# ekinakyurek/Long-Term-Recurrent-Convolutional-NN

Hardware: AMD Instinct MI355X
Metric: training images/sec (VGG16+LSTM, COCO, batch 256) at 1/2/4/8 MI355X (higher is better)
Workload: dtype bf16

## Files before the change

long-term-recurrent-convolutional-nn_amd/_lib.py:

```python
import ctypes as C
import os
import subprocess

HERE = os.path.dirname(os.path.abspath(__file__))
CSRC = os.path.join(HERE, "csrc")
LIB_PATH = os.environ.get("LRCN_HIP_LIB") or os.path.join(CSRC, "liblrcn_hip.so")
HEADER = os.path.normpath(os.path.join(HERE, "..", "include", "lrcn.h"))
SAMPLE_HEADER = os.path.normpath(os.path.join(HERE, "..", "include", "lrcn_sample.h"))
SCORE_HEADER = os.path.normpath(os.path.join(HERE, "..", "include", "lrcn_score.h"))
NUCLEUS_HEADER = os.path.normpath(os.path.join(HERE, "..", "include", "lrcn_nucleus.h"))
NBEST_HEADER = os.path.normpath(os.path.join(HERE, "..", "include", "lrcn_nbest.h"))
DIVERSE_HEADER = os.path.normpath(os.path.join(HERE, "..", "include", "lrcn_diverse.h"))
CONSTRAIN_HEADER = os.path.normpath(os.path.join(HERE, "..", "include", "lrcn_constrain.h"))
ACTIVITY_HEADER = os.path.normpath(os.path.join(HERE, "..", "include", "lrcn_activity.h"))
ACT_DROPOUT_HEADER = os.path.normpath(os.path.join(HERE, "..", "include", "lrcn_act_dropout.h"))
VARLEN_HEADER = os.path.normpath(os.path.join(HERE, "..", "include", "lrcn_varlen.h"))
CLIP_HEADER = os.path.normpath(os.path.join(HERE, "..", "include", "lrcn_clip.h"))
WEIGHTED_HEADER = os.path.normpath(os.path.join(HERE, "..", "include", "lrcn_weighted.h"))
SCHED_HEADER = os.path.normpath(os.path.join(HERE, "..", "include", "lrcn_sched.h"))
SMOOTH_HEADER = os.path.normpath(os.path.join(HERE, "..", "include", "lrcn_smooth.h"))
GEMM_DEBUG_HEADER = os.path.normpath(os.path.join(HERE, "..", "include", "lrcn_gemm_debug.h"))
CONV_DEBUG_HEADER = os.path.normpath(os.path.join(HERE, "..", "include", "lrcn_conv_debug.h"))
DECODE_DEBUG_HEADER = os.path.normpath(os.path.join(HERE, "..", "include", "lrcn_decode_debug.h"))

LRCN_F32, LRCN_BF16, LRCN_FP8 = 0, 1, 2
LRCN_ABI_VERSION = 5
LRCN_OPT_FUSED_UPDATE, LRCN_OPT_DETERMINISTIC, LRCN_OPT_CONV_CHUNK_BYTES = 1, 2, 3
SEGMENTS = ("update", "rec_fwd", "rec_bwd", "embed_gather", "embed_grad", "preprocess", "upload")
EOS, BOS, UNK = 0, 1, 2
CNNOUT = 4096
MAX_T = 28


class LrcnError(RuntimeError):
    pass


class Config(C.Structure):
# ... 256 lines not shown
    "lrcn_debug_conv_gemm": (C.c_int, [C.c_void_p, C.POINTER(ConvGemmDebug)]),
}

CONV_DEBUG_SIGNATURES = {
    "lrcn_debug_conv11": (C.c_int, [C.c_void_p, C.c_void_p, C.c_int, C.c_int, C.c_int, C.POINTER(C.c_float), C.c_void_p, C.c_void_p, C.c_void_p]),
    "lrcn_debug_fp8_cast": (C.c_int, [C.c_void_p, C.c_int, C.c_void_p, C.c_int64, C.c_float, C.c_void_p]),
    "lrcn_debug_amax": (C.c_int, [C.c_void_p, C.c_void_p, C.c_int64, C.c_void_p]),
    "lrcn_debug_conv64_f8": (C.c_int, [C.c_void_p, C.c_void_p, C.c_int, C.c_int, C.c_int, C.c_void_p, C.c_void_p, C.c_int, C.c_float, C.c_void_p]),
    "lrcn_debug_fp8_scales": (C.c_int, [C.c_void_p, C.POINTER(C.c_float)]),
}

DECODE_DEBUG_SIGNATURES = {
    "lrcn_debug_decode_steps": (C.c_int, [C.c_void_p, C.POINTER(DecodeDebug)]),
}


def build(force=False):
    srcs = [os.path.join(CSRC, f) for f in os.listdir(CSRC) if f.endswith((".hip", ".h"))] + [HEADER, SAMPLE_HEADER, NUCLEUS_HEADER, SCORE_HEADER, NBEST_HEADER, DIVERSE_HEADER, CONSTRAIN_HEADER,
                                                                                                   ACTIVITY_HEADER, ACT_DROPOUT_HEADER, VARLEN_HEADER, CLIP_HEADER, WEIGHTED_HEADER, SCHED_HEADER, SMOOTH_HEADER, GEMM_DEBUG_HEADER, CONV_DEBUG_HEADER, DECODE_DEBUG_HEADER]
    stale = force or not os.path.exists(LIB_PATH) or os.path.getmtime(LIB_PATH) < max(os.path.getmtime(s) for s in srcs)
    if stale:
        subprocess.check_call(["make", "-s", "-j4", "-C", CSRC, "-f", os.path.join(CSRC, "Makefile")])
    return LIB_PATH


_LIB = None


def lib():
    global _LIB
    if _LIB is None:
        if not os.path.exists(LIB_PATH):
            raise LrcnError("%s is missing: run `python -c 'import __graft_entry__ as g; g.build()'` "
                            "(there is no CPU fallback)" % LIB_PATH)
        import torch
        L = C.CDLL(LIB_PATH)
        for name, (res, args) in list(SIGNATURES.items()) + list(SAMPLE_SIGNATURES.items()) + list(NUCLEUS_SIGNATURES.items()) + list(SCORE_SIGNATURES.items()) + list(NBEST_SIGNATURES.items()) + list(DIVERSE_SIGNATURES.items()) + list(CONSTRAIN_SIGNATURES.items()) + \
                list(ACTIVITY_SIGNATURES.items()) + list(ACT_DROPOUT_SIGNATURES.items()) + list(VARLEN_SIGNATURES.items()) + list(CLIP_SIGNATURES.items()) + list(WEIGHTED_SIGNATURES.items()) + list(SCHED_SIGNATURES.items()) + list(SMOOTH_SIGNATURES.items()) + \
                list(GEMM_DEBUG_SIGNATURES.items()) + list(CONV_DEBUG_SIGNATURES.items()) + list(DECODE_DEBUG_SIGNATURES.items()):
            fn = getattr(L, name)
            fn.restype = res
            fn.argtypes = args
        if L.lrcn_abi_version() != LRCN_ABI_VERSION:
            raise LrcnError("%s implements ABI revision %d, this binding was written against %d (lrcn_config's layout differs)"
                            % (LIB_PATH, L.lrcn_abi_version(), LRCN_ABI_VERSION))
        _LIB = L
    return _LIB


def check(ctx_handle, rc):
    if rc != 0:
        msg = lib().lrcn_last_error(ctx_handle)
        raise LrcnError("liblrcn_hip error %d: %s" % (rc, msg.decode() if msg else "?"))
```

long-term-recurrent-convolutional-nn_amd/csrc/ctx.h:

```cpp
#pragma once
#include <utility>

#include "comm.h"
#include "host.h"
#include "../../include/lrcn_smooth.h"

namespace lrcn_impl {

struct VggLayer {
    void *w = nullptr;
    void *w_fused = nullptr;
    float *b = nullptr;
    int Cin = 0, Cout = 0, S = 0, pool = 0;
    void *w8 = nullptr;
    float *sw = nullptr, *escale = nullptr, *ebias = nullptr;
};
constexpr int kFp8First = 3;

}

struct lrcn_ctx {
    lrcn_config cfg{};
    hipStream_t stream = nullptr;
    std::string err;
// ... 81 lines not shown
    void *cn_arena = nullptr;
    size_t cn_bytes = 0;
    void *sc_arena = nullptr;
    size_t sc_bytes = 0;
    int ncu = 0;
    int vgg_wg_cap = 0;
    bool vgg_loaded = false;
    bool vgg_fp8 = false, fp8_ready = false;
    float *amax_dev = nullptr;
    float act_scale[13] = {};
    lrcn_impl::VggLayer conv[13];
    void *fc6w = nullptr, *fc7w = nullptr;
    float *fc6b = nullptr, *fc7b = nullptr;
    void *actA = nullptr, *actB = nullptr, *im2col = nullptr, *f6 = nullptr, *img16 = nullptr;
    float *featsRM = nullptr;
    bool prof = false;
    std::vector<std::pair<hipEvent_t, hipEvent_t>> prof_ev;
    size_t prof_used = 0;
    double prof_ms = 0.0;
    int64_t prof_launches = 0;
    int prof_level = 0;
    struct SegProf {
        std::vector<std::pair<hipEvent_t, hipEvent_t>> ev;
        size_t used = 0;
        double ms = 0.0, bytes = 0.0;
        int64_t n = 0;
    } seg[LRCN_SEG_COUNT];
    std::string vgg_routes;
    float *avg_img = nullptr;
    bool avg_on = false;
// ... 106 lines not shown
```

long-term-recurrent-convolutional-nn_amd/csrc/lrcn_api.hip:

```cpp
#include <algorithm>
#include <cmath>

#include "ctx.h"

static thread_local std::string g_create_err;
using namespace lrcn_impl;

constexpr int kBgWgsPerFreeCu = 4;

int lrcn_impl::gemm(lrcn_ctx *c, int dtype, const void *A, int64_t lda, const void *B, int64_t ldb, void *C, int64_t ldc, int M, int N,
         int K, const float *bias, bool c_f32, bool beta, bool relu, bool c_is_zero, bool on_wg_stream) {
    GemmArgs g{};
    g.dtype = dtype;
    g.A = A;
    g.lda = lda;
    g.B = B;
    g.ldb = ldb;
    g.C = C;
    g.ldc = ldc;
    g.M = M;
    g.N = N;
    g.K = gemm_k(dtype, lda, ldb, K);
    g.bias = bias;
    g.c_f32 = c_f32;
// ... 134 lines not shown
    if (c->wg_done) (void)hipEventDestroy(c->wg_done);
    if (c->xc_fork) (void)hipEventDestroy(c->xc_fork);
    if (c->xc_done) (void)hipEventDestroy(c->xc_done);
    if (c->pin) (void)hipHostFree(c->pin);
    if (c->lens_pin) (void)hipHostFree(c->lens_pin);
    for (auto &e : c->lens_up)
        if (e) (void)hipEventDestroy(e);
    if (c->roww_pin) (void)hipHostFree(c->roww_pin);
    for (auto &e : c->roww_up)
        if (e) (void)hipEventDestroy(e);
    if (c->wg_stream && c->wg_stream_owned) (void)hipStreamDestroy(c->wg_stream);
    if (c->copy_stream) (void)hipStreamDestroy(c->copy_stream);
    for (int j = 0; j < lrcn_ctx::kStage; ++j) {
        if (c->up_done[j]) (void)hipEventDestroy(c->up_done[j]);
        if (c->rd_done[j]) (void)hipEventDestroy(c->rd_done[j]);
    }
    comm_destroy(c->comm);
    for (auto &e : c->bucket_done)
        if (e) (void)hipEventDestroy(e);
    for (auto &e : c->ar_done)
        if (e) (void)hipEventDestroy(e);
    if (c->comm_stream && c->comm_stream_owned) (void)hipStreamDestroy(c->comm_stream);
    for (auto &sp : c->seg)
        for (auto &e : sp.ev) {
            (void)hipEventDestroy(e.first);
            (void)hipEventDestroy(e.second);
        }
    for (auto &e : c->prof_ev) {
        (void)hipEventDestroy(e.first);
        (void)hipEventDestroy(e.second);
// ... 324 lines not shown
```

long-term-recurrent-convolutional-nn_amd/csrc/train.hip:

```cpp
#include <cmath>
#include <cstring>

#include "ctx.h"
#include "../../include/lrcn_varlen.h"
#include "../../include/lrcn_clip.h"
#include "../../include/lrcn_weighted.h"
#include "../../include/lrcn_sched.h"
#include "../../include/lrcn_smooth.h"

using namespace lrcn_impl;

namespace {

DropSpec make_drop(const lrcn_dropout *d, int which) {
    DropSpec s{};
    s.which = which;
    if (d) {
        s.p = d->pdrop;
        s.seed = d->seed;
        s.mask = which == 1 ? d->mask1 : d->mask2;
        if (s.mask) s.p = 0.0f;
    }
    return s;
}
// ... 63 lines not shown
            g.out_mode = GEMM_OUT_LSTM_BWD;
            g.lstm.H = H; g.lstm.ld_a = ld4H;
            g.lstm.acts = const_cast<char *>(boff(acts, (int64_t)(s - 1) * B * ld4H, c->esz));
            g.lstm.c_prev = s > 1 ? Call + (int64_t)(s - 2) * B * H : nullptr;
            g.lstm.c_new = Call + (int64_t)(s - 1) * B * H;
            g.lstm.dh_ext = dHall + (int64_t)(s - 1) * B * H;
            g.lstm.dc = c->dc;
            g.lstm.dz_out = boff(dZ, (int64_t)(s - 1) * B * ld4H, c->esz);
            hipError_t e = launch_gemm_8p(c->stream, g);
            if (e != hipSuccess) FAIL(c, LRCN_EHIP, "lstm bwd step (GEMM + cell epilogue): %s", hipGetErrorString(e));
        }
        KCHK(c, "lstm_layer_bwd (epilogue)");
        return LRCN_OK;
    }
    {
        const int nsl = knob_int("LRCN_BWD_SLABS", 0);
        const int Kp = (int)round_up64(4 * H, 64);
        if (!fused && nsl >= 2 && nsl <= 8 && dt == GEMM_T_BF16 && !lstm_alone(c) && bg_row_window(B) && !(H & 3) && H >= 128 &&
            Kp / 64 >= 8 * nsl && Kp <= ld4H && (size_t)nsl * B * H * sizeof(float) <= c->gemm_ws_bytes && c->gemm_ws) {
            float *slabs = reinterpret_cast<float *>(c->gemm_ws);
            for (int s = S - 1; s >= 0; --s) {
                k_lstm_bwd(c->stream, dt, boff(acts, (int64_t)s * B * ld4H, c->esz), ld4H, s ? Call + (int64_t)(s - 1) * B * H : nullptr,
                           Call + (int64_t)s * B * H, dHall + (int64_t)s * B * H, H, slabs, s < S - 1, c->dc, s == S - 1, B, H,
                           boff(dZ, (int64_t)s * B * ld4H, c->esz), ld4H, nsl);
                if (s > 0) {
                    GemmArgs g = rec_step_args(c, dZ, ld4H, s, B, WhT, H, Kp);
                    g.C = slabs; g.ldc = H; g.c_f32 = 1;
                    g.out_mode = GEMM_OUT_PLAIN;
                    g.ws = c->gemm_ws; g.ws_bytes = c->gemm_ws_bytes;
                    g.cfg_pref = 2;
                    g.splitk_forced = 1; g.splitk_no_reduce = 1;
// ... 600 lines not shown
```

long-term-recurrent-convolutional-nn_amd/csrc/vgg.hip:

```cpp
#include <algorithm>
#include <cstring>

#include "ctx.h"
#include "../../include/lrcn_conv_debug.h"
#include "../../include/lrcn_gemm_debug.h"

using namespace lrcn_impl;

static const int kVggCout[13] = {64, 64, 128, 128, 256, 256, 256, 512, 512, 512, 512, 512, 512};
static const int kVggPool[13] = {0, 1, 0, 1, 0, 0, 1, 0, 0, 1, 0, 0, 1};

namespace {
int stamps_reserve(lrcn_ctx *c, int64_t need) {
    if (need > c->stamps_n) {
        c->stamps = nullptr;
        DALLOC(c, c->stamps, sizeof(unsigned long long) * (size_t)need);
        c->stamps_n = need;
    }
    return LRCN_OK;
}
bool conv64_enabled() { return !knob_off("LRCN_CONV64"); }
constexpr int kTileCtrStride = 8 + 2 * 512;
hipError_t launch_conv_chunked(hipStream_t st, const GemmArgs &g0, int N, int es, int64_t limit_bytes = 0) {
    const int64_t per_img = (int64_t)g0.H * g0.W * g0.Cin * es;
// ... 66 lines not shown

int conv_layer_fp8(lrcn_ctx *c, const void *in, const VggLayer &L, int N, void *out, int *tile_ctr = nullptr) {
    GemmArgs g = conv_args(c, GEMM_T_F8, in, L, N, out, tile_ctr);
    g.B = L.w8;
    g.bias = L.ebias;
    g.scale = L.escale;
    hipError_t e = launch_conv_chunked(c->stream, g, N, 1, c->conv_chunk_bytes > 0 ? c->conv_chunk_bytes : 0x7F000000ll);
    if (e != hipSuccess) FAIL(c, LRCN_EHIP, "fp8 conv layer S=%d Cin=%d Cout=%d: %s", L.S, L.Cin, L.Cout, hipGetErrorString(e));
    return LRCN_OK;
}

}

namespace lrcn_impl {

int vgg_body(lrcn_ctx *c, int N, const void *src, bool src_u8, const float *mean, bool calibrate) {
    const bool fp8 = c->vgg_fp8 && !calibrate;
    if (fp8 && !c->fp8_ready) FAIL(c, LRCN_ESTATE, "vgg_dtype = LRCN_FP8: call lrcn_vgg_calibrate before the first forward");
    const int vdt = c->vdt;
    const float m0 = mean ? mean[0] : 0.f, m1 = mean ? mean[1] : 0.f, m2 = mean ? mean[2] : 0.f;
    const bool fuse11 = vdt == GEMM_T_BF16 && src_u8 && c->conv[0].w_fused && conv64_enabled() && !knob_off("LRCN_FUSE11");
    const float *avg = (src_u8 && c->avg_on) ? c->avg_img : nullptr;
    int staged = -1;
    if (src_u8)
        for (int j = 0; j < lrcn_ctx::kStage; ++j)
            if (c->stage[j] && src == c->stage[j]) staged = j;
    if (staged >= 0) HIPCHK(c, hipStreamWaitEvent(c->stream, c->up_done[staged], 0));
    auto crops_consumed = [&]() -> int {
        if (staged < 0) return LRCN_OK;
        HIPCHK(c, hipEventRecord(c->rd_done[staged], c->stream));
        c->stage_read[staged] = true;
// ... 40 lines not shown
        g.out_mode = GEMM_OUT_CONV;
        g.H = g.W = 224;
        g.zero_page = c->zero_page;
        hipError_t e = launch_gemm(c->stream, g);
        if (e != hipSuccess) FAIL(c, LRCN_EHIP, "conv1_1: %s", hipGetErrorString(e));
    }
    if (int r = crops_consumed()) return r;
    if (!fuse11) note(vdt == GEMM_T_BF16 ? "conv11" : gemm_debug_last_route());
    void *cur = c->actA, *nxt = c->actB;
    int *ctr = nullptr;
    if (c->vgg_wg_cap >= 8 && knob_char("LRCN_DYN_TILES") == '1') {
        if (!c->tile_ctr) DALLOC(c, c->tile_ctr, sizeof(int) * 13 * kTileCtrStride);
        HIPCHK(c, hipMemsetAsync(c->tile_ctr, 0, sizeof(int) * 13 * kTileCtrStride, c->stream));
        ctr = c->tile_ctr;
    }
    std::pair<hipEvent_t, hipEvent_t> *ev = nullptr;
    if (c->prof) {
        if (c->prof_used == c->prof_ev.size()) {
            std::pair<hipEvent_t, hipEvent_t> e;
            HIPCHK(c, hipEventCreate(&e.first));
            HIPCHK(c, hipEventCreate(&e.second));
            c->prof_ev.push_back(e);
        }
        ev = &c->prof_ev[c->prof_used++];
        HIPCHK(c, hipEventRecord(ev->first, c->stream));
    }
    int l0 = 1;
    if (fuse11) {
        unsigned long long *stamps = nullptr;
        if (knob_char("LRCN_STAMPS") == 'f') {
            if (int r = stamps_reserve(c, (int64_t)N * 14 * 14 * 16)) return r;
            stamps = c->stamps;
        }
        hipError_t e = launch_conv64_fused11(c->stream, c->img16, c->conv[0].w_fused, c->conv[0].b, c->conv[1].w, c->conv[1].b, nxt, N, 224,
                                             c->zero_page, c->vgg_wg_cap, stamps);
        if (e != hipSuccess) FAIL(c, LRCN_EHIP, "fused conv1_1+conv1_2: %s", hipGetErrorString(e));
        note(gemm_debug_last_route());
        std::swap(cur, nxt);
        l0 = 2;
    }
    auto out_count = [&](int l) {
        const VggLayer &L = c->conv[l];
        const int64_t So = L.pool ? L.S / 2 : L.S;
        return (int64_t)N * So * So * L.Cout;
    };
    bool in_is_f8 = false;
    for (int l = l0; l < 13; ++l) {
        if (fp8 && l == kFp8First && !in_is_f8) {
            k_cast_bf16_fp8(c->stream, cur, out_count(l - 1), 1.0f / c->act_scale[l - 1], nxt);
            std::swap(cur, nxt);
        }
        int r;
        if (fp8 && l >= kFp8First)
            r = conv_layer_fp8(c, cur, c->conv[l], N, nxt, ctr ? ctr + l * kTileCtrStride : nullptr);
        else
            r = conv_layer(c, vdt, cur, c->conv[l], N, nxt, (fp8 && l == kFp8First - 1) ? 1.0f / c->act_scale[l] : 0.0f, &in_is_f8,
                           ctr ? ctr + l * kTileCtrStride : nullptr);
        if (r) return r;
        note(gemm_debug_last_route());
        std::swap(cur, nxt);
        if (calibrate && l >= kFp8First - 1) k_amax(c->stream, cur, out_count(l), c->amax_dev + l);
    }
    if (fp8) {
        k_cast_fp8_bf16(c->stream, cur, out_count(12), c->act_scale[12], nxt);
        std::swap(cur, nxt);
    }
    if (ev) HIPCHK(c, hipEventRecord(ev->second, c->stream));
    GemmArgs g{};
    g.dtype = vdt;
    g.A = cur;
    g.lda = 25088;
    g.B = c->fc6w;
    g.ldb = 25088;
    g.M = N;
    g.N = 4096;
    g.K = 25088;
    g.zero_page = c->zero_page;
    g.ws = c->vgg_ws;
    g.ws_bytes = c->gemm_ws_bytes;
    g.C = c->f6;
    g.ldc = 4096;
    g.bias = c->fc6b;
    g.relu = 1;
    hipError_t e = launch_gemm(c->stream, g);
    if (e != hipSuccess) FAIL(c, LRCN_EHIP, "fc6: %s", hipGetErrorString(e));
    note(gemm_debug_last_route());
    g.A = c->f6;
    g.lda = 4096;
    g.B = c->fc7w;
    g.ldb = 4096;
    g.C = c->featsRM;
    g.K = 4096;
    g.bias = c->fc7b;
    g.relu = 0;
    g.c_f32 = 1;
    e = launch_gemm(c->stream, g);
    if (e != hipSuccess) FAIL(c, LRCN_EHIP, "fc7: %s", hipGetErrorString(e));
    note(gemm_debug_last_route());
    return LRCN_OK;
}
int vgg_check(lrcn_ctx *c, int N) {
    if (!c->vgg_loaded) FAIL(c, LRCN_ESTATE, "lrcn_vgg_load has not been called");
    if (N < 1 || N > c->cfg.max_images) FAIL(c, LRCN_EINVAL, "N=%d outside [1,%d]", N, c->cfg.max_images);
    return LRCN_OK;
}
}

extern "C" {

int lrcn_vgg_load(lrcn_ctx *c, const float *const cw[13], const float *const cb[13], const float *fc6_w, const float *fc6_b,
                  const float *fc7_w, const float *fc7_b) {
    DeviceGuard dg(c);
    if (!c || !cw || !cb || !fc6_w || !fc6_b || !fc7_w || !fc7_b) return LRCN_EINVAL;
    if (c->cfg.max_images < 1) FAIL(c, LRCN_ESTATE, "context was created with max_images = 0");
// ... 269 lines not shown
    if (!c || !img || !feats || (!mean && !c->avg_on)) return LRCN_EINVAL;
    int r = vgg_check(c, N);
    if (r) return r;
    if (block_rows < 1 || N % block_rows) FAIL(c, LRCN_EINVAL, "block_rows=%d must divide N=%d", block_rows, N);
    r = vgg_body(c, N, img, true, mean);
    if (r) return r;
    for (int b = 0; b < N / block_rows; ++b) {
        float *dst = feats + (int64_t)b * block_rows * LRCN_CNNOUT;
        k_transpose_f32(c->stream, c->featsRM + (int64_t)b * block_rows * LRCN_CNNOUT, 4096, block_rows, 4096, dst, block_rows);
        if (normalize) k_normalize_rows(c->stream, dst, block_rows, LRCN_CNNOUT);
    }
    KCHK(c, "vgg_forward_u8_blocks");
    return LRCN_OK;
}

int lrcn_preprocess_u8(lrcn_ctx *c, const uint8_t *img, int N, const float mean[3], float *out) {
    DeviceGuard dg(c);
    if (!c || !img || !out || (!mean && !c->avg_on) || N < 1) return LRCN_EINVAL;
    k_preprocess_u8(c->stream, img, N, 224, mean ? mean[0] : 0.f, mean ? mean[1] : 0.f, mean ? mean[2] : 0.f, c->avg_on ? c->avg_img : nullptr, out);
    KCHK(c, "preprocess_u8");
    return LRCN_OK;
}

int lrcn_set_average_image(lrcn_ctx *c, const float *avg) {
    DeviceGuard dg(c);
    if (!c) return LRCN_EINVAL;
    if (!avg) {
        c->avg_on = false;
        return LRCN_OK;
    }
// ... 337 lines not shown
```

long-term-recurrent-convolutional-nn_amd/dp.py:

```python
import collections
import ctypes as C
import os

import numpy as np
import torch
import torch.distributed as dist

from . import lrcn as L


def shard_rows(B_global, world, rank):
    if B_global % world:
        raise L.LrcnError("global batch %d is not divisible by world size %d" % (B_global, world))
    b = B_global // world
    return slice(rank * b, (rank + 1) * b)


def vgg_wg_cap_for(device, rows=256, chunk=1):
    ncu = torch.cuda.get_device_properties(device).multi_processor_count
    if chunk > 1 and rows <= 32:
        return (ncu * 5 // 8) & ~7
    if chunk > 1 and rows <= 64:
        return (ncu * 11 // 16) & ~7
    return (ncu * 7 // 8) & ~7
# ... 53 lines not shown

class HipOps:

    def __init__(self, ctx, mean=L.VGG_MEAN):
        self.ctx = ctx
        self.mean = mean

    def vgg(self, img_u8, feats=None, normalize=False):
        return L.convnet_u8(self.ctx, img_u8, mean=self.mean, feats=feats, normalize=normalize)

    def loss(self, param, feats, tokens, lens=None):
        return L.avg_loss_batch(self.ctx, param, feats, tokens, lens=lens)

    def vgg_blocks(self, img_u8, rows, feats=None, normalize=False):
        return L.convnet_u8_blocks(self.ctx, img_u8, rows, mean=self.mean, feats=feats, normalize=normalize)

    def upload(self, host_u8):
        return L.upload_crops(self.ctx, host_u8)

    def params_touched(self):
        self.ctx.params_touched()

    def side_stream(self):
        if os.environ.get("LRCN_OVERLAP_VGG", "1")[:1] == "0":
            return None
        prio = int(os.environ.get("LRCN_VGG_STREAM_PRIO", "0"))
        return torch.cuda.Stream(device=self.ctx.device, priority=prio)

    def set_vgg_wg_cap(self, cap):
        self.ctx._call("lrcn_vgg_set_wg_cap", int(cap))
# ... 144 lines not shown
            self._v = [torch.zeros(n, device=dev, dtype=torch.float32) for n in n_of]
            self._gshard = [torch.zeros(n, device=dev, dtype=torch.float32) for n in n_of]
            self._scatter_optim_state()
        else:
            self.flat_grads, self.grads = flat_model_like(shapes, device=param[0].device)
        self.step_no = 0
        self._feat_q = collections.deque()
        self._chunk_no = 0
        self._side = self.ops.side_stream() if hasattr(self.ops, "side_stream") else None
        if self._side is not None and hasattr(self.ops, "set_vgg_wg_cap"):
            env = os.environ.get("LRCN_VGG_WG_CAP")
            cap = int(env) if env is not None else vgg_wg_cap_for(param[0].device, int(rows) if rows else B_global // max(world, 1), int(vgg_chunk))
            self.ops.set_vgg_wg_cap(cap)
            self.vgg_cap = cap
        self._feats_buf = [None, None]
        if (self._side is not None and isinstance(self._side, torch.cuda.Stream) and ctx is not None and hasattr(self.ops, "set_wg_stream")
                and os.environ.get("LRCN_DP_WG_STREAM_PROBE", "1")[:1] != "0"):
            self.ops.set_wg_stream(avoid=[self._side, torch.cuda.current_stream(ctx.device)])
        self._bucket_streams = None
        self._abi_stream_set = False
        env_sp = os.environ.get("LRCN_DP_SPARSE_EMBED")
        want = (env_sp[:1] != "0") if env_sp else world > 1
        self._sparse_embed = bool(want and self.backend == "torch" and not self.shard and not host_clip and self._multi_or_forced_sparse(env_sp)
                                  and hasattr(self.ops, "embed_grad_from_rows") and hasattr(self.ops, "update_group") and ctx is not None
                                  and self._group_pipeline())
        if self._sparse_embed:
            W = max(world, 1)
            cap = (ctx.max_T + 1) * min(ctx.max_B, int(rows) if rows else ctx.max_B)
            if W * cap > 8192:
                self._sparse_embed = False
# ... 203 lines not shown
        return self.ops.vgg(img_u8, normalize=True) if self.normalize_features else self.ops.vgg(img_u8)

    def _vgg_blocks(self, img_u8, rows, out=None):
        if img_u8.shape[0] == rows or not hasattr(self.ops, "vgg_blocks"):
            if img_u8.shape[0] != rows:
                raise L.LrcnError("crops for %d rows given, the step has %d (these ops cannot run several batches in one forward)" % (img_u8.shape[0], rows))
            return [self.ops.vgg(img_u8, feats=out, normalize=True) if self.normalize_features else self.ops.vgg(img_u8, feats=out)]
        if img_u8.shape[0] % rows:
            raise L.LrcnError("crops for %d rows are not a whole number of %d-row batches" % (img_u8.shape[0], rows))
        return self.ops.vgg_blocks(img_u8, rows, feats=out, normalize=self.normalize_features)

    def _vgg_on_side_stream(self, img_u8, rows):
        main = torch.cuda.current_stream(self.ctx.device)
        k = self._chunk_no & 1
        self._chunk_no += 1
        n = img_u8.shape[0] * L.CNNOUT
        if self._feats_buf[k] is None or self._feats_buf[k].numel() != n:
            self._feats_buf[k] = (torch.empty(n, device=self.param[0].device, dtype=torch.float32) if img_u8.shape[0] != rows
                                  else L.jl_empty(rows, L.CNNOUT))
        self._side.wait_stream(main)
        self.ctx.use_stream(self._side)
        try:
            blocks = self._vgg_blocks(img_u8, rows, out=self._feats_buf[k])
        finally:
            self.ctx.use_stream(main)
        if torch.is_tensor(img_u8) and img_u8.is_cuda:
            img_u8.record_stream(self._side)
        ev = torch.cuda.Event()
        ev.record(self._side)
        for b in blocks:
# ... 17 lines not shown
        if label_smoothing > 0:
            if self.backend == "abi" and self._multi:
                raise L.LrcnError("the \"abi\" data-parallel backend (lrcn_train_step_dp) has no label smoothing; use backend=\"torch\"")
            if lens is None:
                lens = np.full(rows, int(tokens.shape[0]), np.int32)
                norm_tokens = self.B_global * (int(tokens.shape[0]) + 1)
        if sched is not None:
            if self.backend == "abi" and self._multi:
                raise L.LrcnError("the \"abi\" data-parallel backend (lrcn_train_step_dp) has no scheduled sampling; use backend=\"torch\"")
            eps, temperature, sseed = tuple(sched)[:3]
            sched = (eps, temperature, sseed, shard_rows(self.B_global, self.world, self.rank).start)
            if lens is None:
                lens = np.full(rows, int(tokens.shape[0]), np.int32)
                norm_tokens = self.B_global * (int(tokens.shape[0]) + 1)
        self._cur_M = (int(tokens.shape[0]) + 1) * rows
        if feats is None:
            if self._feat_q:
                feats, ev = self._feat_q.popleft()
                if ev is not None:
                    torch.cuda.current_stream(self.ctx.device).wait_event(ev)
            else:
                blocks = self._vgg_blocks(self._device_crops(img_u8), rows)
                feats = blocks[0]
                self._feat_q.extend((b, None) for b in blocks[1:])
        self.step_no += 1
        consumed, deferred = False, None
        if next_img_u8 is not None and len(self._feat_q) < max(1, next_img_u8.shape[0] // rows):
            consumed = True
            nxt = self._device_crops(next_img_u8)
            if self._side is not None:
                self._vgg_on_side_stream(nxt, rows)
            else:
                deferred = nxt
            if prefetch_img_u8 is not None and hasattr(self.ops, "upload") and torch.is_tensor(prefetch_img_u8) and not prefetch_img_u8.is_cuda:
                self._prefetched = (prefetch_img_u8, self.ops.upload(prefetch_img_u8))

        def inorder_vgg():
            if deferred is not None:
                self._feat_q.extend((b, None) for b in self._vgg_blocks(deferred, rows))
# ... 158 lines not shown
            else:
                parts = [torch.empty_like(mine) for _ in range(self._W)]
                dist.all_gather(parts, mine.clone(), group=self.group)
                for i, t in enumerate(parts):
                    self.flat_param[a + i * n:a + (i + 1) * n].copy_(t)
        if self._shadow_groups:
            self.ops.refresh_shadows_group(self.param, k, s)

    def describe(self):
        buckets = os.environ.get("LRCN_DP_BUCKETS", "1")[:1] != "0"
        return {"backend": self.backend, "update": "sharded" if self.shard else "replicated", "fused_update": bool(self._fused),
                "shadows_by_group": bool(getattr(self, "_shadow_groups", False)),
                "per_group_pipeline": bool(self.shard or (self.backend == "abi" and self._multi) or self._group_pipeline()),
                "one_allreduce_of_the_flat_buffer": bool(self.world > 1 and not buckets and not self.shard),
                "sparse_embedding_exchange": bool(getattr(self, "_sparse_embed", False)), "vgg_side_stream": self._side is not None,
                "queue_probe": getattr(self, "queue_probe", None), "backend_note": self.backend_note or None,
                "update_stream_on_its_own_queue": getattr(self.ops, "update_stream_probed", None)}

    def _dist_on(self):
        return dist.is_available() and dist.is_initialized()

    def _gather_cat(self, t):
        if not self._dist_on():
            return t.clone()
        W = dist.get_world_size(self.group)
        if dist.get_backend(self.group) == "nccl":
            out = torch.empty((W,) + tuple(t.shape), device=t.device, dtype=t.dtype)
            dist.all_gather_into_tensor(out, t.contiguous(), group=self.group)
            return out.view((W * t.shape[0],) + tuple(t.shape[1:]))
        h = t.detach().cpu().contiguous()
# ... 84 lines not shown
```

long-term-recurrent-convolutional-nn_amd/launch.py:

```python
import json
import os
import signal
import socket
import subprocess
import sys
import tempfile
import time


def find_free_port():
    with socket.socket() as sk:
        sk.bind(("127.0.0.1", 0))
        return sk.getsockname()[1]


def run_ranks(script, argv, nranks, env_extra=None, watchdog_s=900.0, capture=True):
    env = dict(os.environ)
    env.setdefault("HSA_ENABLE_IPC_MODE_LEGACY", "0")
    env.update(env_extra or {})
    cmd = [sys.executable, "-m", "torch.distributed.run", "--nnodes=1", "--nproc-per-node", str(nranks), "--master-addr", "127.0.0.1",
           "--master-port", str(find_free_port()), os.path.abspath(script)] + list(argv)
    proc = subprocess.Popen(cmd, env=env, stdout=subprocess.PIPE if capture else None, stderr=None, text=True, start_new_session=True)

    def stop_job():
# ... 20 lines not shown
            rc = proc.returncode
        except subprocess.TimeoutExpired:
            stop_job()
            out, _ = proc.communicate()
            rc = 124
    finally:
        stop_job()
        for sg, h in old.items():
            signal.signal(sg, h)
    return rc, out


PLAIN_ENV = {
    "LRCN_DP_BACKEND": "torch", "LRCN_DP_SHARD_ADAM": "0", "LRCN_DP_SPARSE_EMBED": "0", "LRCN_DP_BUCKETS": "0", "LRCN_DP_GROUP_ADAM": "0",
    "LRCN_DP_QUEUE_PROBE": "0", "LRCN_DP_WG_STREAM_PROBE": "0", "LRCN_FUSED_UPDATE": "0", "LRCN_VGG_CHUNK_IMAGES": "0",
}


def default_rungs(dp_backend="torch"):
    rungs = []
    if dp_backend == "auto":
        rungs.append(("abi", {"LRCN_DP_BACKEND": "abi"}))
    rungs.append(("default", {"LRCN_DP_BACKEND": "abi" if dp_backend == "abi" else "torch"}))
    rungs.append(("plain", dict(PLAIN_ENV)))
    return rungs


def _set_pdeathsig():
    try:
        import ctypes
# ... 176 lines not shown
```

long-term-recurrent-convolutional-nn_amd/lrcn.py:

```python
import ctypes as C

import numpy as np
import torch

from . import _lib
from ._lib import BOS, CNNOUT, EOS, LRCN_BF16, LRCN_F32, LRCN_FP8, UNK, LrcnError

PARAM_NAMES = ("W1", "b1", "W2", "b2", "Wproj", "Wcnn", "Wembed", "Wout", "bout")
VGG_COUT = (64, 64, 128, 128, 256, 256, 256, 512, 512, 512, 512, 512, 512)
VGG_MEAN = (123.68, 116.779, 103.939)


def jl_empty(*dims, device="cuda", dtype=torch.float32):
    t = torch.empty(tuple(reversed(dims)), device=device, dtype=dtype)
    return t.permute(*reversed(range(len(dims))))


def jl_zeros(*dims, device="cuda", dtype=torch.float32):
    t = jl_empty(*dims, device=device, dtype=dtype)
    t.zero_()
    return t


def to_jl(a, device="cuda"):
# ... 739 lines not shown


def convnet_u8_blocks(ctx, img_u8, block_rows, mean=VGG_MEAN, feats=None, normalize=False):
    if torch.is_tensor(img_u8) and not img_u8.is_cuda:
        img_u8 = upload_crops(ctx, img_u8)
    N = img_u8.shape[0]
    m = N // block_rows
    if feats is None:
        feats = torch.empty(m * block_rows * CNNOUT, device="cuda", dtype=torch.float32)
    mm = (C.c_float * 3)(*mean) if mean is not None else None
    ctx._call("lrcn_vgg_forward_u8_blocks", C.c_void_p(img_u8.data_ptr()), N, mm, int(block_rows), int(bool(normalize)), C.c_void_p(feats.data_ptr()))
    n = block_rows * CNNOUT
    return [feats[b * n:(b + 1) * n].view(CNNOUT, block_rows).permute(1, 0) for b in range(m)]


class StagedCrops:

    def __init__(self, ptr, N, host):
        self.ptr, self.shape, self.host = int(ptr), (int(N), 224, 224, 3), host
        self.is_cuda = True

    def data_ptr(self):
        return self.ptr


def upload_crops(ctx, host_u8):
    if host_u8.is_cuda or host_u8.dtype != torch.uint8 or not host_u8.is_contiguous() or tuple(host_u8.shape[1:]) != (224, 224, 3):
        raise LrcnError("upload_crops takes a contiguous CPU uint8 tensor [N][224][224][3]")
    out = C.c_void_p()
    ctx._call("lrcn_upload_crops", C.c_void_p(host_u8.data_ptr()), int(host_u8.shape[0]), C.byref(out))
# ... 217 lines not shown
```

Measured before the change: 37200.

## Split VGG forward into side-stream convolutions and main-stream FC head with double-buffered pool5

Splits the VGG forward into a convolution part issued on the side stream and an fc6/fc7 head issued on the main stream, using two pool5 buffers tracked by filled/freed events. When both buffers are full, the last conv layer is held back and launched after the head frees its buffer. The aim is to overlap the next batch's convolutions with the current step's LSTM work, so the main stream no longer waits on the whole VGG. The change also turns LSTM backward slabs on by default (LRCN_BWD_SLABS 0→4). In exchange it adds buffer memory, cross-stream event bookkeeping and more complex state that can be misordered.

```diff
diff --git a/include/lrcn_vgg_split.h b/include/lrcn_vgg_split.h
--- /dev/null
+++ b/include/lrcn_vgg_split.h
@@ -0,0 +1,18 @@
+#ifndef LRCN_VGG_SPLIT_H
+#define LRCN_VGG_SPLIT_H
+
+#include "lrcn.h"
+
+#ifdef __cplusplus
+extern "C" {
+#endif
+
+int lrcn_vgg_convs_u8(lrcn_ctx *ctx, const uint8_t *img, int N, const float mean[3], int *block_out);
+
+int lrcn_vgg_head(lrcn_ctx *ctx, int block, void *stream, float *feats);
+
+#ifdef __cplusplus
+}
+#endif
+
+#endif
diff --git a/long-term-recurrent-convolutional-nn_amd/_lib.py b/long-term-recurrent-convolutional-nn_amd/_lib.py
--- a/long-term-recurrent-convolutional-nn_amd/_lib.py
+++ b/long-term-recurrent-convolutional-nn_amd/_lib.py
@@ -22,6 +22,7 @@
 GEMM_DEBUG_HEADER = os.path.normpath(os.path.join(HERE, "..", "include", "lrcn_gemm_debug.h"))
 CONV_DEBUG_HEADER = os.path.normpath(os.path.join(HERE, "..", "include", "lrcn_conv_debug.h"))
 DECODE_DEBUG_HEADER = os.path.normpath(os.path.join(HERE, "..", "include", "lrcn_decode_debug.h"))
+VGG_SPLIT_HEADER = os.path.normpath(os.path.join(HERE, "..", "include", "lrcn_vgg_split.h"))
 
 LRCN_F32, LRCN_BF16, LRCN_FP8 = 0, 1, 2
 LRCN_ABI_VERSION = 5
@@ -308,10 +309,15 @@
     "lrcn_debug_decode_steps": (C.c_int, [C.c_void_p, C.POINTER(DecodeDebug)]),
 }
 
+VGG_SPLIT_SIGNATURES = {
+    "lrcn_vgg_convs_u8": (C.c_int, [C.c_void_p, C.c_void_p, C.c_int, C.POINTER(C.c_float), C.POINTER(C.c_int)]),
+    "lrcn_vgg_head": (C.c_int, [C.c_void_p, C.c_int, C.c_void_p, C.c_void_p]),
+}
+
 
 def build(force=False):
     srcs = [os.path.join(CSRC, f) for f in os.listdir(CSRC) if f.endswith((".hip", ".h"))] + [HEADER, SAMPLE_HEADER, NUCLEUS_HEADER, SCORE_HEADER, NBEST_HEADER, DIVERSE_HEADER, CONSTRAIN_HEADER,
-                                                                                                   ACTIVITY_HEADER, ACT_DROPOUT_HEADER, VARLEN_HEADER, CLIP_HEADER, WEIGHTED_HEADER, SCHED_HEADER, SMOOTH_HEADER, GEMM_DEBUG_HEADER, CONV_DEBUG_HEADER, DECODE_DEBUG_HEADER]
+                                                                                                   ACTIVITY_HEADER, ACT_DROPOUT_HEADER, VARLEN_HEADER, CLIP_HEADER, WEIGHTED_HEADER, SCHED_HEADER, SMOOTH_HEADER, GEMM_DEBUG_HEADER, CONV_DEBUG_HEADER, DECODE_DEBUG_HEADER, VGG_SPLIT_HEADER]
     stale = force or not os.path.exists(LIB_PATH) or os.path.getmtime(LIB_PATH) < max(os.path.getmtime(s) for s in srcs)
     if stale:
         subprocess.check_call(["make", "-s", "-j4", "-C", CSRC, "-f", os.path.join(CSRC, "Makefile")])
@@ -331,7 +337,7 @@
         L = C.CDLL(LIB_PATH)
         for name, (res, args) in list(SIGNATURES.items()) + list(SAMPLE_SIGNATURES.items()) + list(NUCLEUS_SIGNATURES.items()) + list(SCORE_SIGNATURES.items()) + list(NBEST_SIGNATURES.items()) + list(DIVERSE_SIGNATURES.items()) + list(CONSTRAIN_SIGNATURES.items()) + \
                 list(ACTIVITY_SIGNATURES.items()) + list(ACT_DROPOUT_SIGNATURES.items()) + list(VARLEN_SIGNATURES.items()) + list(CLIP_SIGNATURES.items()) + list(WEIGHTED_SIGNATURES.items()) + list(SCHED_SIGNATURES.items()) + list(SMOOTH_SIGNATURES.items()) + \
-                list(GEMM_DEBUG_SIGNATURES.items()) + list(CONV_DEBUG_SIGNATURES.items()) + list(DECODE_DEBUG_SIGNATURES.items()):
+                list(GEMM_DEBUG_SIGNATURES.items()) + list(CONV_DEBUG_SIGNATURES.items()) + list(DECODE_DEBUG_SIGNATURES.items()) + list(VGG_SPLIT_SIGNATURES.items()):
             fn = getattr(L, name)
             fn.restype = res
             fn.argtypes = args
diff --git a/long-term-recurrent-convolutional-nn_amd/csrc/ctx.h b/long-term-recurrent-convolutional-nn_amd/csrc/ctx.h
--- a/long-term-recurrent-convolutional-nn_amd/csrc/ctx.h
+++ b/long-term-recurrent-convolutional-nn_amd/csrc/ctx.h
@@ -119,6 +119,21 @@
     float *fc6b = nullptr, *fc7b = nullptr;
     void *actA = nullptr, *actB = nullptr, *im2col = nullptr, *f6 = nullptr, *img16 = nullptr;
     float *featsRM = nullptr;
+    struct Pool5Block {
+        void *buf = nullptr;
+        hipEvent_t filled = nullptr, freed = nullptr;
+        int N = 0;
+        bool full = false;
+        bool read = false;
+    } p5[2];
+    int p5_next = 0;
+    struct Pool5Held {
+        bool on = false;
+        int block = 0, N = 0;
+        const void *in = nullptr;
+        hipStream_t st = nullptr;
+        long prof_slot = -1;
+    } p5_held;
     bool prof = false;
     std::vector<std::pair<hipEvent_t, hipEvent_t>> prof_ev;
     size_t prof_used = 0;
diff --git a/long-term-recurrent-convolutional-nn_amd/csrc/lrcn_api.hip b/long-term-recurrent-convolutional-nn_amd/csrc/lrcn_api.hip
--- a/long-term-recurrent-convolutional-nn_amd/csrc/lrcn_api.hip
+++ b/long-term-recurrent-convolutional-nn_amd/csrc/lrcn_api.hip
@@ -172,6 +172,10 @@
     for (int j = 0; j < lrcn_ctx::kStage; ++j) {
         if (c->up_done[j]) (void)hipEventDestroy(c->up_done[j]);
         if (c->rd_done[j]) (void)hipEventDestroy(c->rd_done[j]);
+    }
+    for (auto &P : c->p5) {
+        if (P.filled) (void)hipEventDestroy(P.filled);
+        if (P.freed) (void)hipEventDestroy(P.freed);
     }
     comm_destroy(c->comm);
     for (auto &e : c->bucket_done)
diff --git a/long-term-recurrent-convolutional-nn_amd/csrc/train.hip b/long-term-recurrent-convolutional-nn_amd/csrc/train.hip
--- a/long-term-recurrent-convolutional-nn_amd/csrc/train.hip
+++ b/long-term-recurrent-convolutional-nn_amd/csrc/train.hip
@@ -101,7 +101,7 @@
         return LRCN_OK;
     }
     {
-        const int nsl = knob_int("LRCN_BWD_SLABS", 0);
+        const int nsl = knob_int("LRCN_BWD_SLABS", 4);
         const int Kp = (int)round_up64(4 * H, 64);
         if (!fused && nsl >= 2 && nsl <= 8 && dt == GEMM_T_BF16 && !lstm_alone(c) && bg_row_window(B) && !(H & 3) && H >= 128 &&
             Kp / 64 >= 8 * nsl && Kp <= ld4H && (size_t)nsl * B * H * sizeof(float) <= c->gemm_ws_bytes && c->gemm_ws) {
diff --git a/long-term-recurrent-convolutional-nn_amd/csrc/vgg.hip b/long-term-recurrent-convolutional-nn_amd/csrc/vgg.hip
--- a/long-term-recurrent-convolutional-nn_amd/csrc/vgg.hip
+++ b/long-term-recurrent-convolutional-nn_amd/csrc/vgg.hip
@@ -4,6 +4,7 @@
 #include "ctx.h"
 #include "../../include/lrcn_conv_debug.h"
 #include "../../include/lrcn_gemm_debug.h"
+#include "../../include/lrcn_vgg_split.h"
 
 using namespace lrcn_impl;
 
@@ -104,7 +105,9 @@
 
 namespace lrcn_impl {
 
-int vgg_body(lrcn_ctx *c, int N, const void *src, bool src_u8, const float *mean, bool calibrate) {
+static int vgg_convs(lrcn_ctx *c, int N, const void *src, bool src_u8, const float *mean, bool calibrate, void *pool5_dst, bool hold_last,
+                     const void **pool5) {
+    if (c->p5_held.on) FAIL(c, LRCN_ESTATE, "a convolution part is waiting for the head of pool5 block %d: issue lrcn_vgg_head first", c->p5_held.block);
     const bool fp8 = c->vgg_fp8 && !calibrate;
     if (fp8 && !c->fp8_ready) FAIL(c, LRCN_ESTATE, "vgg_dtype = LRCN_FP8: call lrcn_vgg_calibrate before the first forward");
     const int vdt = c->vdt;
@@ -175,7 +178,7 @@
         HIPCHK(c, hipMemsetAsync(c->tile_ctr, 0, sizeof(int) * 13 * kTileCtrStride, c->stream));
         ctr = c->tile_ctr;
     }
-    std::pair<hipEvent_t, hipEvent_t> *ev = nullptr;
+    long prof_slot = -1;
     if (c->prof) {
         if (c->prof_used == c->prof_ev.size()) {
             std::pair<hipEvent_t, hipEvent_t> e;
@@ -183,8 +186,8 @@
             HIPCHK(c, hipEventCreate(&e.second));
             c->prof_ev.push_back(e);
         }
-        ev = &c->prof_ev[c->prof_used++];
-        HIPCHK(c, hipEventRecord(ev->first, c->stream));
+        prof_slot = (long)c->prof_used++;
+        HIPCHK(c, hipEventRecord(c->prof_ev[prof_slot].first, c->stream));
     }
     int l0 = 1;
     if (fuse11) {
@@ -211,25 +214,62 @@
             k_cast_bf16_fp8(c->stream, cur, out_count(l - 1), 1.0f / c->act_scale[l - 1], nxt);
             std::swap(cur, nxt);
         }
+        if (l == 12 && hold_last) {
+            c->p5_held.in = cur;
+            c->p5_held.N = N;
+            c->p5_held.st = c->stream;
+            c->p5_held.prof_slot = prof_slot;
+            c->p5_held.on = true;
+            return LRCN_OK;
+        }
+        void *out = (l == 12 && pool5_dst) ? pool5_dst : nxt;
         int r;
         if (fp8 && l >= kFp8First)
-            r = conv_layer_fp8(c, cur, c->conv[l], N, nxt, ctr ? ctr + l * kTileCtrStride : nullptr);
+            r = conv_layer_fp8(c, cur, c->conv[l], N, out, ctr ? ctr + l * kTileCtrStride : nullptr);
         else
-            r = conv_layer(c, vdt, cur, c->conv[l], N, nxt, (fp8 && l == kFp8First - 1) ? 1.0f / c->act_scale[l] : 0.0f, &in_is_f8,
+            r = conv_layer(c, vdt, cur, c->conv[l], N, out, (fp8 && l == kFp8First - 1) ? 1.0f / c->act_scale[l] : 0.0f, &in_is_f8,
                            ctr ? ctr + l * kTileCtrStride : nullptr);
         if (r) return r;
         note(gemm_debug_last_route());
-        std::swap(cur, nxt);
+        if (out == nxt)
+            std::swap(cur, nxt);
+        else
+            cur = out;
         if (calibrate && l >= kFp8First - 1) k_amax(c->stream, cur, out_count(l), c->amax_dev + l);
     }
     if (fp8) {
         k_cast_fp8_bf16(c->stream, cur, out_count(12), c->act_scale[12], nxt);
         std::swap(cur, nxt);
     }
-    if (ev) HIPCHK(c, hipEventRecord(ev->second, c->stream));
+    if (prof_slot >= 0) HIPCHK(c, hipEventRecord(c->prof_ev[prof_slot].second, c->stream));
+    *pool5 = cur;
+    return LRCN_OK;
+}
+
+static int launch_held_conv53(lrcn_ctx *c, void *pool5_dst) {
+    lrcn_ctx::Pool5Held &h = c->p5_held;
+    h.on = false;
+    hipStream_t keep = c->stream;
+    c->stream = h.st;
+    const int r = conv_layer(c, c->vdt, h.in, c->conv[12], h.N, pool5_dst);
+    hipError_t e = hipSuccess;
+    if (!r && h.prof_slot >= 0) e = hipEventRecord(c->prof_ev[h.prof_slot].second, h.st);
+    c->stream = keep;
+    if (r) return r;
+    HIPCHK(c, e);
+    c->vgg_routes += ',';
+    c->vgg_routes += gemm_debug_last_route();
+    return LRCN_OK;
+}
+
+static int vgg_head(lrcn_ctx *c, hipStream_t st, const void *pool5, int N, void *ws) {
+    auto note = [&](const char *r) {
+        if (!c->vgg_routes.empty()) c->vgg_routes += ',';
+        c->vgg_routes += r;
+    };
     GemmArgs g{};
-    g.dtype = vdt;
-    g.A = cur;
+    g.dtype = c->vdt;
+    g.A = pool5;
     g.lda = 25088;
     g.B = c->fc6w;
     g.ldb = 25088;
@@ -237,13 +277,13 @@
     g.N = 4096;
     g.K = 25088;
     g.zero_page = c->zero_page;
-    g.ws = c->vgg_ws;
-    g.ws_bytes = c->gemm_ws_bytes;
+    g.ws = ws;
+    g.ws_bytes = ws ? c->gemm_ws_bytes : 0;
     g.C = c->f6;
     g.ldc = 4096;
     g.bias = c->fc6b;
     g.relu = 1;
-    hipError_t e = launch_gemm(c->stream, g);
+    hipError_t e = launch_gemm(st, g);
     if (e != hipSuccess) FAIL(c, LRCN_EHIP, "fc6: %s", hipGetErrorString(e));
     note(gemm_debug_last_route());
     g.A = c->f6;
@@ -255,10 +295,16 @@
     g.bias = c->fc7b;
     g.relu = 0;
     g.c_f32 = 1;
-    e = launch_gemm(c->stream, g);
+    e = launch_gemm(st, g);
     if (e != hipSuccess) FAIL(c, LRCN_EHIP, "fc7: %s", hipGetErrorString(e));
     note(gemm_debug_last_route());
     return LRCN_OK;
+}
+
+int vgg_body(lrcn_ctx *c, int N, const void *src, bool src_u8, const float *mean, bool calibrate) {
+    const void *pool5 = nullptr;
+    if (int r = vgg_convs(c, N, src, src_u8, mean, calibrate, nullptr, false, &pool5)) return r;
+    return vgg_head(c, c->stream, pool5, N, c->vgg_ws);
 }
 int vgg_check(lrcn_ctx *c, int N) {
     if (!c->vgg_loaded) FAIL(c, LRCN_ESTATE, "lrcn_vgg_load has not been called");
@@ -558,6 +604,71 @@
     return LRCN_OK;
 }
 
+static int split_check(lrcn_ctx *c) {
+    if (c->vdt != GEMM_T_BF16 || c->vgg_fp8) FAIL(c, LRCN_EINVAL, "the two-call VGG forward needs vgg_dtype = LRCN_BF16");
+    return LRCN_OK;
+}
+
+int lrcn_vgg_convs_u8(lrcn_ctx *c, const uint8_t *img, int N, const float mean[3], int *block_out) {
+    DeviceGuard dg(c);
+    if (!c || !img || !block_out || (!mean && !c->avg_on)) return LRCN_EINVAL;
+    int r = vgg_check(c, N);
+    if (r) return r;
+    if ((r = split_check(c))) return r;
+    for (auto &P : c->p5) {
+        if (!P.buf) DALLOC(c, P.buf, 2 * (size_t)c->cfg.max_images * 25088);
+        if (!P.filled) HIPCHK(c, hipEventCreateWithFlags(&P.filled, hipEventDisableTiming));
+        if (!P.freed) HIPCHK(c, hipEventCreateWithFlags(&P.freed, hipEventDisableTiming));
+    }
+    const int b = c->p5_next;
+    lrcn_ctx::Pool5Block &P = c->p5[b];
+    const bool hold = P.full;
+    if (!hold && P.read) HIPCHK(c, hipStreamWaitEvent(c->stream, P.freed, 0));
+    const void *pool5 = nullptr;
+    if ((r = vgg_convs(c, N, img, true, mean, false, P.buf, hold, &pool5))) return r;
+    if (hold) {
+        c->p5_held.block = b;
+    } else {
+        HIPCHK(c, hipEventRecord(P.filled, c->stream));
+        P.N = N;
+        P.full = true;
+    }
+    c->p5_next = b ^ 1;
+    *block_out = b;
+    KCHK(c, "vgg_convs_u8");
+    return LRCN_OK;
+}
+
+int lrcn_vgg_head(lrcn_ctx *c, int block, void *stream, float *feats) {
+    DeviceGuard dg(c);
+    if (!c || !feats) return LRCN_EINVAL;
+    if (!c->vgg_loaded) FAIL(c, LRCN_ESTATE, "lrcn_vgg_load has not been called");
+    int r = split_check(c);
+    if (r) return r;
+    if (block < 0 || block > 1) FAIL(c, LRCN_EINVAL, "block=%d outside [0,1]", block);
+    lrcn_ctx::Pool5Block &P = c->p5[block];
+    if (!P.full) FAIL(c, LRCN_ESTATE, "pool5 block %d holds no features: no convolution part has been issued into it since its last head", block);
+    hipStream_t st = stream_or_ctx(c, stream);
+    HIPCHK(c, hipStreamWaitEvent(st, P.filled, 0));
+    c->vgg_routes.clear();
+    if ((r = vgg_head(c, st, P.buf, P.N, c->gemm_ws))) return r;
+    k_transpose_f32(st, c->featsRM, 4096, P.N, 4096, feats, P.N);
+    HIPCHK(c, hipEventRecord(P.freed, st));
+    P.full = false;
+    P.read = true;
+    if (c->p5_held.on && c->p5_held.block == block) {
+        HIPCHK(c, hipStreamWaitEvent(c->p5_held.st, P.freed, 0));
+        const int heldN = c->p5_held.N;
+        hipStream_t held_st = c->p5_held.st;
+        if ((r = launch_held_conv53(c, P.buf))) return r;
+        HIPCHK(c, hipEventRecord(P.filled, held_st));
+        P.N = heldN;
+        P.full = true;
+    }
+    KCHK(c, "vgg_head");
+    return LRCN_OK;
+}
+
 int lrcn_preprocess_u8(lrcn_ctx *c, const uint8_t *img, int N, const float mean[3], float *out) {
     DeviceGuard dg(c);
     if (!c || !img || !out || (!mean && !c->avg_on) || N < 1) return LRCN_EINVAL;
diff --git a/long-term-recurrent-convolutional-nn_amd/dp.py b/long-term-recurrent-convolutional-nn_amd/dp.py
--- a/long-term-recurrent-convolutional-nn_amd/dp.py
+++ b/long-term-recurrent-convolutional-nn_amd/dp.py
@@ -91,6 +91,12 @@
 
     def vgg_blocks(self, img_u8, rows, feats=None, normalize=False):
         return L.convnet_u8_blocks(self.ctx, img_u8, rows, mean=self.mean, feats=feats, normalize=normalize)
+
+    def vgg_convs(self, img_u8):
+        return L.vgg_convs_u8(self.ctx, img_u8, mean=self.mean)
+
+    def vgg_head(self, block, n, feats, stream, normalize=False):
+        return L.vgg_head(self.ctx, block, n, feats=feats, stream=stream, normalize=normalize)
 
     def upload(self, host_u8):
         return L.upload_crops(self.ctx, host_u8)
@@ -265,6 +271,11 @@
             self.ops.set_vgg_wg_cap(cap)
             self.vgg_cap = cap
         self._feats_buf = [None, None]
+        rows_here = int(rows) if rows else B_global // max(world, 1)
+        self._split_head = bool(self._side is not None and isinstance(self._side, torch.cuda.Stream) and ctx is not None
+                                and hasattr(self.ops, "vgg_convs") and 256 <= rows_here <= 512 and int(vgg_chunk) == 1
+                                and getattr(ctx, "vgg_dtype", None) == L.LRCN_BF16
+                                and os.environ.get("LRCN_DP_SPLIT_HEAD", "1")[:1] != "0")
         if (self._side is not None and isinstance(self._side, torch.cuda.Stream) and ctx is not None and hasattr(self.ops, "set_wg_stream")
                 and os.environ.get("LRCN_DP_WG_STREAM_PROBE", "1")[:1] != "0"):
             self.ops.set_wg_stream(avoid=[self._side, torch.cuda.current_stream(ctx.device)])
@@ -498,6 +509,19 @@
         main = torch.cuda.current_stream(self.ctx.device)
         k = self._chunk_no & 1
         self._chunk_no += 1
+        if self._split_head and img_u8.shape[0] == rows:
+            self._side.wait_event(self._step_begin)
+            self.ctx.use_stream(self._side)
+            try:
+                block, n_img = self.ops.vgg_convs(img_u8)
+            finally:
+                self.ctx.use_stream(main)
+            if torch.is_tensor(img_u8) and img_u8.is_cuda:
+                img_u8.record_stream(self._side)
+            if self._feats_buf[k] is None or self._feats_buf[k].numel() != rows * L.CNNOUT:
+                self._feats_buf[k] = L.jl_empty(rows, L.CNNOUT)
+            self._feat_q.append((self._feats_buf[k], ("head", block, n_img)))
+            return
         n = img_u8.shape[0] * L.CNNOUT
         if self._feats_buf[k] is None or self._feats_buf[k].numel() != n:
             self._feats_buf[k] = (torch.empty(n, device=self.param[0].device, dtype=torch.float32) if img_u8.shape[0] != rows
@@ -545,15 +569,22 @@
                 lens = np.full(rows, int(tokens.shape[0]), np.int32)
                 norm_tokens = self.B_global * (int(tokens.shape[0]) + 1)
         self._cur_M = (int(tokens.shape[0]) + 1) * rows
+        if self._split_head:
+            self._step_begin = torch.cuda.Event()
+            self._step_begin.record(torch.cuda.current_stream(self.ctx.device))
         if feats is None:
             if self._feat_q:
                 feats, ev = self._feat_q.popleft()
-                if ev is not None:
+                if isinstance(ev, tuple):
+                    self.ops.vgg_head(ev[1], ev[2], feats, torch.cuda.current_stream(self.ctx.device), normalize=self.normalize_features)
+                elif ev is not None:
                     torch.cuda.current_stream(self.ctx.device).wait_event(ev)
             else:
                 blocks = self._vgg_blocks(self._device_crops(img_u8), rows)
                 feats = blocks[0]
                 self._feat_q.extend((b, None) for b in blocks[1:])
+                if self._split_head:
+                    self._step_begin.record(torch.cuda.current_stream(self.ctx.device))
         self.step_no += 1
         consumed, deferred = False, None
         if next_img_u8 is not None and len(self._feat_q) < max(1, next_img_u8.shape[0] // rows):
@@ -742,6 +773,7 @@
                 "per_group_pipeline": bool(self.shard or (self.backend == "abi" and self._multi) or self._group_pipeline()),
                 "one_allreduce_of_the_flat_buffer": bool(self.world > 1 and not buckets and not self.shard),
                 "sparse_embedding_exchange": bool(getattr(self, "_sparse_embed", False)), "vgg_side_stream": self._side is not None,
+                "vgg_forward": "convolutions on the side stream, head on the main stream" if getattr(self, "_split_head", False) else "one call",
                 "queue_probe": getattr(self, "queue_probe", None), "backend_note": self.backend_note or None,
                 "update_stream_on_its_own_queue": getattr(self.ops, "update_stream_probed", None)}
 
diff --git a/long-term-recurrent-convolutional-nn_amd/launch.py b/long-term-recurrent-convolutional-nn_amd/launch.py
--- a/long-term-recurrent-convolutional-nn_amd/launch.py
+++ b/long-term-recurrent-convolutional-nn_amd/launch.py
@@ -58,6 +58,7 @@
 PLAIN_ENV = {
     "LRCN_DP_BACKEND": "torch", "LRCN_DP_SHARD_ADAM": "0", "LRCN_DP_SPARSE_EMBED": "0", "LRCN_DP_BUCKETS": "0", "LRCN_DP_GROUP_ADAM": "0",
     "LRCN_DP_QUEUE_PROBE": "0", "LRCN_DP_WG_STREAM_PROBE": "0", "LRCN_FUSED_UPDATE": "0", "LRCN_VGG_CHUNK_IMAGES": "0",
+    "LRCN_DP_SPLIT_HEAD": "0",
 }
 
 
diff --git a/long-term-recurrent-convolutional-nn_amd/lrcn.py b/long-term-recurrent-convolutional-nn_amd/lrcn.py
--- a/long-term-recurrent-convolutional-nn_amd/lrcn.py
+++ b/long-term-recurrent-convolutional-nn_amd/lrcn.py
@@ -777,6 +777,25 @@
     return [feats[b * n:(b + 1) * n].view(CNNOUT, block_rows).permute(1, 0) for b in range(m)]
 
 
+def vgg_convs_u8(ctx, img_u8, mean=VGG_MEAN):
+    if torch.is_tensor(img_u8) and not img_u8.is_cuda:
+        img_u8 = upload_crops(ctx, img_u8)
+    N = img_u8.shape[0]
+    m = (C.c_float * 3)(*mean) if mean is not None else None
+    block = C.c_int(-1)
+    ctx._call("lrcn_vgg_convs_u8", C.c_void_p(img_u8.data_ptr()), N, m, C.byref(block))
+    return block.value, N
+
+
+def vgg_head(ctx, block, N, feats=None, stream=None, normalize=False):
+    if feats is None:
+        feats = jl_empty(N, CNNOUT)
+    ctx._call("lrcn_vgg_head", int(block), _stream_arg(stream), _ptr(feats))
+    if normalize:
+        normalize_features(ctx, feats)
+    return feats
+
+
 class StagedCrops:
 
     def __init__(self, ptr, N, host):
```

Result: no change. 37110 (-0.2%).
